# maybeLx/MVSFormerPlusPlus

Hardware: AMD Instinct MI355X
Metric: ref-views/sec at 1152x1536 N=5 D=192 4-stage; achieved HBM GB/s vs peak (higher is better)
Workload: dtype fp16 operands/storage, fp32 accumulate (every stage; 1-2 fp16 MFMA terms)

## Files before the change

### mvsformerplusplus_amd/csrc/conv_bf16x3_kernels.hip

```cpp
#include <map>
#include <mutex>
#include <type_traits>
#include <utility>

#include "conv_cfg.h"
#include "split_format.h"

namespace mvs {

template <class Base>
struct F16Cfg : Base { static constexpr int ACT_F16 = 1; };
template <class Base>
struct F16x1Cfg : Base { static constexpr int ACT_F16 = 2; };
template <class Cfg, class = void> struct CfgFmt { static constexpr bool F16 = false, ONE = false; };
template <class Cfg> struct CfgFmt<Cfg, decltype((void)Cfg::ACT_F16)> { static constexpr bool F16 = true, ONE = Cfg::ACT_F16 == 2; };
typedef _Float16 f16x8 __attribute__((ext_vector_type(8)));
typedef _Float16 f16x4 __attribute__((ext_vector_type(4)));

__device__ __forceinline__ f16x4 f16_pack4(const float4& v, float& amax) {
    const float m = 65504.0f;
    sat::track(amax, v.x, v.y, v.z, v.w);
    return f16x4{(_Float16)__builtin_amdgcn_fmed3f(v.x, -m, m), (_Float16)__builtin_amdgcn_fmed3f(v.y, -m, m),
                 (_Float16)__builtin_amdgcn_fmed3f(v.z, -m, m), (_Float16)__builtin_amdgcn_fmed3f(v.w, -m, m)};
}

__device__ __forceinline__ float4 f16_quad_to_f32(const float4& raw) {
    const float lo = raw.x, hi = raw.y;
    const f16x4 h = __builtin_bit_cast(f16x4, make_float2(lo, hi));
    return make_float4((float)h[0], (float)h[1], (float)h[2], (float)h[3]);
}

template <int MREP, int NREP, bool F16 = false, bool ONE = false>
__device__ __forceinline__ void bf_mfma_step(const bf16x8* ah, const bf16x8* al, const bf16x8* bh, const bf16x8* bl, f32x4 (*acc)[NREP]) {
    if constexpr (F16) {
        if constexpr (!ONE) {
#pragma unroll
            for (int mb = 0; mb < MREP; ++mb)
#pragma unroll
                for (int nb = 0; nb < NREP; ++nb)
                    acc[mb][nb] = __builtin_amdgcn_mfma_f32_16x16x32_f16(__builtin_bit_cast(f16x8, al[mb]), __builtin_bit_cast(f16x8, bh[nb]), acc[mb][nb], 0, 0, 0);
        }
#pragma unroll
        for (int mb = 0; mb < MREP; ++mb)
#pragma unroll
            for (int nb = 0; nb < NREP; ++nb)
                acc[mb][nb] = __builtin_amdgcn_mfma_f32_16x16x32_f16(__builtin_bit_cast(f16x8, ah[mb]), __builtin_bit_cast(f16x8, bh[nb]), acc[mb][nb], 0, 0, 0);
        return;
    }
#pragma unroll
    for (int mb = 0; mb < MREP; ++mb)
#pragma unroll
        for (int nb = 0; nb < NREP; ++nb) acc[mb][nb] = __builtin_amdgcn_mfma_f32_16x16x32_bf16(al[mb], bh[nb], acc[mb][nb], 0, 0, 0);
#pragma unroll
    for (int mb = 0; mb < MREP; ++mb)
#pragma unroll
        for (int nb = 0; nb < NREP; ++nb) acc[mb][nb] = __builtin_amdgcn_mfma_f32_16x16x32_bf16(ah[mb], bl[nb], acc[mb][nb], 0, 0, 0);
#pragma unroll
    for (int mb = 0; mb < MREP; ++mb)
#pragma unroll
        for (int nb = 0; nb < NREP; ++nb) acc[mb][nb] = __builtin_amdgcn_mfma_f32_16x16x32_bf16(ah[mb], bh[nb], acc[mb][nb], 0, 0, 0);
}

template <class Base, int MSPLIT_>
struct SplitCfg : Base {
    static constexpr int MSPLIT = MSPLIT_;
    static constexpr int MREP_ALL = Base::MREP;
    static constexpr int MREP = Base::MREP / MSPLIT_;
    static constexpr int NREP = Base::NREP * MSPLIT_;
    static_assert(Base::MREP % MSPLIT_ == 0 && 4 % MSPLIT_ == 0, "bad output-block split");
};
template <class Cfg, class = void> struct CfgSplit { static constexpr int MSPLIT = 1, MREP_ALL = Cfg::MREP; };
template <class Cfg> struct CfgSplit<Cfg, decltype((void)Cfg::MSPLIT)> { static constexpr int MSPLIT = Cfg::MSPLIT, MREP_ALL = Cfg::MREP_ALL; };

constexpr int bf_f16_plane_shift(int sw) { return sw == 1 ? 0 : 16; }

template <class Cfg>
struct BfConv {
    static constexpr int OPT = Cfg::CH / 8;
    static constexpr int NSTEP = (Cfg::NTAP * OPT + 3) / 4;
    static constexpr bool PLANES = OPT == 2;
    static constexpr bool F16 = CfgFmt<Cfg>::F16;
    static constexpr int RUNB = F16 ? 16 : 32;
    static constexpr int SB = F16 ? 16 : (PLANES ? 32 : Cfg::S * 4);
    static constexpr int PLANE = F16 ? (Cfg::NVOX * 16 + 255) / 256 * 256 + bf_f16_plane_shift(Cfg::SW)
                                     : (PLANES ? (Cfg::NVOX * 32 + 255) / 256 * 256 + 16 : 32);
    static constexpr size_t LDS_BYTES = F16 ? (size_t)OPT * PLANE : (PLANES ? (size_t)2 * PLANE : Cfg::LDS_BYTES);
    static constexpr bool ONE = CfgFmt<Cfg>::ONE;
    static constexpr bool PERSIST = (Cfg::CIN == 8 || ONE) && Cfg::NPASS == 1 && NSTEP * Cfg::MREP * (ONE ? 4 : 8) <= 64;
    static constexpr bool PERSIST_WLDS = PERSIST && ONE && Cfg::CIN == 16;
    static constexpr int WLDS_OFF = ((int)LDS_BYTES + 255) / 256 * 256;
    static constexpr size_t PERSIST_LDS_BYTES = PERSIST_WLDS ? (size_t)WLDS_OFF + (size_t)NSTEP * Cfg::MREP * 1024 : LDS_BYTES;
    static constexpr bool UNROLL_STAGE = !(Cfg::CIN == 32 && Cfg::COUT == 32);
    static_assert(Cfg::CH % 8 == 0 && OPT <= 2, "split-bf16 path stages one or two octets per pass");
};

constexpr unsigned BF_OOB = 0x80000000u;

__device__ __forceinline__ __amdgpu_buffer_rsrc_t bf_make_rsrc(const void* p, unsigned bytes) {
    return __builtin_amdgcn_make_buffer_rsrc(const_cast<void*>(p), 0, (int)bytes, 0x00020000);
}
__device__ __forceinline__ __amdgpu_buffer_rsrc_t bf_make_rsrc_z(const char* xb, int z0, int D, int H, int W, unsigned vstride, int& zrel) {
// ... 40 lines not shown
    const int tx = tile % tiles_x;
    const int t1 = tile / tiles_x;
    return {tx, t1 % tiles_y, t1 / tiles_y};
}

template <int MREP, int NREP>
__device__ __forceinline__ void bf_zero_acc(f32x4 (*acc)[NREP]) {
#pragma unroll
    for (int mb = 0; mb < MREP; ++mb)
#pragma unroll
        for (int nb = 0; nb < NREP; ++nb) acc[mb][nb] = (f32x4){0.0f, 0.0f, 0.0f, 0.0f};
}

template <bool F16, bool SPLIT>
__device__ __forceinline__ void bf_store_quad(float* o, int co, int g, const float4& v, bool ok, float& sat_amax) {
    static_assert(!(F16 && SPLIT), "fp16 tensors have no split form: only the split store looks at `ok`");
    if constexpr (F16) *reinterpret_cast<f16x4*>(reinterpret_cast<_Float16*>(o) + co) = f16_pack4(v, sat_amax);
    else if constexpr (SPLIT) split_store_quad(o + (co & ~7), g, v, ok);
    else *reinterpret_cast<float4*>(o + co) = v;
}
template <bool F16, bool SPLIT>
__device__ __forceinline__ void bf_skip_join(float4& v, const float4& raw) {
    const float4 sk = F16 ? f16_quad_to_f32(raw) : SPLIT ? split_join_quad(raw) : raw;
    v.x += sk.x; v.y += sk.y; v.z += sk.z; v.w += sk.w;
}
__device__ __forceinline__ void bf_prob_head(const float4& v, const float4& pw4, float pb, int g, bool ok, float* logits, size_t idx) {
    float part = v.x * pw4.x;
    part += v.y * pw4.y;
    part += v.z * pw4.z;
    part += v.w * pw4.w;
    part += __shfl_xor(part, 16);
    if ((g & 1) == 0 && ok) logits[idx] = part + pb;
}

template <class Cfg>
__device__ __forceinline__ constexpr int bf_tap_offset(int o) {
    constexpr int OPT = BfConv<Cfg>::OPT;
    int tap = o / OPT;
    const int oc = o - tap * OPT;
    tap = tap < Cfg::NTAP ? tap : Cfg::NTAP - 1;
    const int kd = tap / 9, r9 = tap - kd * 9, kh = r9 / 3, kw = r9 - kh * 3;
    return ((kd * Cfg::IH + kh) * Cfg::IW + kw) * BfConv<Cfg>::SB + oc * BfConv<Cfg>::PLANE;
}

template <class Cfg, int T>
__device__ __forceinline__ void bf_conv_load_w(const bf16x8* wq, bf16x8* ah, bf16x8* al) {
#pragma unroll
    for (int mb = 0; mb < Cfg::MREP; ++mb) {
        ah[mb] = wq[(size_t)((T * CfgSplit<Cfg>::MREP_ALL + mb) * 2) * 64];
        al[mb] = wq[(size_t)((T * CfgSplit<Cfg>::MREP_ALL + mb) * 2 + 1) * 64];
    }
}

template <class Cfg, int T>
__device__ __forceinline__ void bf_conv_load_x(int g, const char* ldsb, int voxbase0, bf16x8* bh, bf16x8* bl) {
    static_assert(Cfg::TH % Cfg::NREP == 0, "a wave's rows must stay inside one output plane");
    constexpr int ROWB = Cfg::SH * Cfg::IW * BfConv<Cfg>::SB;
    constexpr int c0 = bf_tap_offset<Cfg>(4 * T), c1 = bf_tap_offset<Cfg>(4 * T + 1), c2 = bf_tap_offset<Cfg>(4 * T + 2),
                  c3 = bf_tap_offset<Cfg>(4 * T + 3);
    int sel;
    if constexpr (BfConv<Cfg>::PLANES) {
        static_assert(c1 == c0 + BfConv<Cfg>::PLANE && c3 == c2 + BfConv<Cfg>::PLANE, "octet planes of one tap");
        sel = ((g & 2) ? c2 : c0) + (g & 1) * BfConv<Cfg>::PLANE;
    } else {
        sel = c0;
        sel = g == 1 ? c1 : sel;
        sel = g == 2 ? c2 : sel;
        sel = g == 3 ? c3 : sel;
    }
    const char* p = ldsb + voxbase0 + sel;
#pragma unroll
    for (int nb = 0; nb < Cfg::NREP; ++nb) {
        bh[nb] = *reinterpret_cast<const bf16x8*>(p + nb * ROWB);
        if constexpr (!BfConv<Cfg>::F16) bl[nb] = *reinterpret_cast<const bf16x8*>(p + nb * ROWB + 16);
    }
}

template <class Cfg, int T>
__device__ __forceinline__ void bf_conv_load_step(int g, const bf16x8* wq, const char* ldsb, int voxbase0, bf16x8* ah, bf16x8* al,
                                                  bf16x8* bh, bf16x8* bl) {
    bf_conv_load_w<Cfg, T>(wq, ah, al);
    bf_conv_load_x<Cfg, T>(g, ldsb, voxbase0, bh, bl);
}

constexpr int BF_WPF = 1;
template <class Cfg, int T>
struct BfConvSteps {
    static constexpr int WPF = BF_WPF, NW = WPF + 1;
    static __device__ __forceinline__ void run(int g, const bf16x8* wq, const char* ldsb, int voxbase0, f32x4 (*acc)[Cfg::NREP],
                                               bf16x8 (*ah)[Cfg::MREP], bf16x8 (*al)[Cfg::MREP], bf16x8* bh0, bf16x8* bl0, bf16x8* bh1, bf16x8* bl1) {
        constexpr int NSTEP = BfConv<Cfg>::NSTEP;
        if constexpr (T < NSTEP) {
            if constexpr (T + WPF < NSTEP) bf_conv_load_w<Cfg, T + WPF>(wq, ah[(T + WPF) % NW], al[(T + WPF) % NW]);
            if constexpr (T + 1 < NSTEP) {
                if constexpr ((T & 1) == 0) bf_conv_load_x<Cfg, T + 1>(g, ldsb, voxbase0, bh1, bl1);
                else bf_conv_load_x<Cfg, T + 1>(g, ldsb, voxbase0, bh0, bl0);
            }
            __builtin_amdgcn_sched_barrier(0);
            if constexpr ((T & 1) == 0) bf_mfma_step<Cfg::MREP, Cfg::NREP, CfgFmt<Cfg>::F16, CfgFmt<Cfg>::ONE>(ah[T % NW], al[T % NW], bh0, bl0, acc);
            else bf_mfma_step<Cfg::MREP, Cfg::NREP, CfgFmt<Cfg>::F16, CfgFmt<Cfg>::ONE>(ah[T % NW], al[T % NW], bh1, bl1, acc);
            BfConvSteps<Cfg, T + 1>::run(g, wq, ldsb, voxbase0, acc, ah, al, bh0, bl0, bh1, bl1);
        }
    }
};

template <class Cfg, int T = 0>
__device__ __forceinline__ void bf_conv_preload_w(const bf16x8* wq, bf16x8 (*ah)[Cfg::MREP], bf16x8 (*al)[Cfg::MREP]) {
    if constexpr (T < BF_WPF && T < BfConv<Cfg>::NSTEP) {
        bf_conv_load_w<Cfg, T>(wq, ah[T], al[T]);
        bf_conv_preload_w<Cfg, T + 1>(wq, ah, al);
    }
}

template <class Cfg>
__device__ __forceinline__ void bf_conv_contract(const bf16x8* wq, const char* ldsb, const int* voxbase, int g, f32x4 (*acc)[Cfg::NREP],
                                                 bf16x8 (*ah)[Cfg::MREP], bf16x8 (*al)[Cfg::MREP]) {
    constexpr int NREP = Cfg::NREP;
    bf16x8 bh0[NREP], bl0[NREP], bh1[NREP], bl1[NREP];
    bf_conv_load_x<Cfg, 0>(g, ldsb, voxbase[0], bh0, bl0);
    BfConvSteps<Cfg, 0>::run(g, wq, ldsb, voxbase[0], acc, ah, al, bh0, bl0, bh1, bl1);
}

template <class Cfg>
struct BfWlds {
    static constexpr int MREP_ALL = CfgSplit<Cfg>::MREP_ALL;
    static constexpr int NSTEP = BfConv<Cfg>::NSTEP;
    static constexpr int WC = (MREP_ALL == 1 && NSTEP % 2 == 0) ? 2 : 1;
    static constexpr int CHUNK_BYTES = WC * MREP_ALL * 2048;
    static constexpr int NPIECE = CHUNK_BYTES / 4096 > 0 ? CHUNK_BYTES / 4096 : 1;
    static constexpr int NCHUNK = NSTEP / WC;
    static constexpr int RING_OFF = ((int)BfConv<Cfg>::LDS_BYTES + 255) / 256 * 256;
    static constexpr size_t LDS_BYTES = (size_t)RING_OFF + 2 * CHUNK_BYTES;
    static constexpr bool ENABLED = !BfConv<Cfg>::PERSIST && NSTEP % WC == 0 && CHUNK_BYTES % 4096 == 0 && MREP_ALL == 1 && WC == 2;
};

struct BfWPiece { float4 a, b; };
template <class Cfg>
__device__ __forceinline__ void bf_wlds_fetch(const void* wp, int gc, int nchunk_total, int tid, BfWPiece& piece) {
    using W = BfWlds<Cfg>;
    static_assert(W::NPIECE <= 2, "at most two pieces per thread and chunk");
    if (gc >= nchunk_total) return;
    const float4* src = reinterpret_cast<const float4*>(reinterpret_cast<const char*>(wp) + (size_t)gc * W::CHUNK_BYTES);
    piece.a = src[tid];
    if constexpr (W::NPIECE > 1) piece.b = src[tid + 256];
}
template <class Cfg>
__device__ __forceinline__ void bf_wlds_store(char* ring, int gc, int tid, const BfWPiece& piece) {
    using W = BfWlds<Cfg>;
    float4* dst = reinterpret_cast<float4*>(ring + (gc & 1) * W::CHUNK_BYTES);
    dst[tid] = piece.a;
    if constexpr (W::NPIECE > 1) dst[tid + 256] = piece.b;
}

template <class Cfg, int T>
__device__ __forceinline__ void bf_wlds_load_a(const char* ring, int gc, int mb0, int lane, bf16x8* ah, bf16x8* al) {
    using W = BfWlds<Cfg>;
    const char* base = ring + (gc & 1) * W::CHUNK_BYTES + ((T % W::WC) * W::MREP_ALL + mb0) * 2048 + lane * 16;
#pragma unroll
    for (int mb = 0; mb < Cfg::MREP; ++mb) {
        ah[mb] = *reinterpret_cast<const bf16x8*>(base + mb * 2048);
        al[mb] = *reinterpret_cast<const bf16x8*>(base + mb * 2048 + 1024);
    }
}

template <class Cfg, int T>
struct BfWldsSteps {
    static __device__ __forceinline__ void run(int g, int lane, int tid, const void* wp, char* ring, int gc0, int nchunk_total, int mb0,
                                               const char* ldsb, int voxbase0, f32x4 (*acc)[Cfg::NREP], BfWPiece& piece, bf16x8* bh0, bf16x8* bl0,
                                               bf16x8* bh1, bf16x8* bl1) {
        using W = BfWlds<Cfg>;
        constexpr int NSTEP = W::NSTEP;
        if constexpr (T < NSTEP) {
            const int gc = gc0 + T / W::WC;
            if constexpr (T % W::WC == 0) bf_wlds_fetch<Cfg>(wp, gc + 1, nchunk_total, tid, piece);
            bf16x8 ah[Cfg::MREP], al[Cfg::MREP];
            bf_wlds_load_a<Cfg, T>(ring, gc, mb0, lane, ah, al);
            if constexpr (T + 1 < NSTEP) {
                if constexpr ((T & 1) == 0) bf_conv_load_x<Cfg, T + 1>(g, ldsb, voxbase0, bh1, bl1);
                else bf_conv_load_x<Cfg, T + 1>(g, ldsb, voxbase0, bh0, bl0);
            }
            __builtin_amdgcn_sched_barrier(0);
            if constexpr ((T & 1) == 0) bf_mfma_step<Cfg::MREP, Cfg::NREP, CfgFmt<Cfg>::F16, CfgFmt<Cfg>::ONE>(ah, al, bh0, bl0, acc);
            else bf_mfma_step<Cfg::MREP, Cfg::NREP, CfgFmt<Cfg>::F16, CfgFmt<Cfg>::ONE>(ah, al, bh1, bl1, acc);
            if constexpr (T % W::WC == W::WC - 1) {
                if (gc + 1 < nchunk_total) bf_wlds_store<Cfg>(ring, gc + 1, tid, piece);
                __syncthreads();
            }
            BfWldsSteps<Cfg, T + 1>::run(g, lane, tid, wp, ring, gc0, nchunk_total, mb0, ldsb, voxbase0, acc, piece, bh0, bl0, bh1, bl1);
        }
    }
};

template <class Cfg, bool SPLIT>
__global__ __launch_bounds__(256) void conv3d_mfma_bf16x3_kernel(const float* __restrict__ x, const void* wp, const float* __restrict__ bias,
                                                                 float* __restrict__ y, int D, int H, int W, int OD, int OH, int OW,
                                                                 int relu, int tiles_x, int tiles_y, int ntiles) {
    float sat_amax = 0.0f;
    constexpr int CIN = Cfg::CIN, COUT = Cfg::COUT, SD = Cfg::SD, SH = Cfg::SH, SW = Cfg::SW, TD = Cfg::TD, TH = Cfg::TH, CH = Cfg::CH;
    constexpr int IH = Cfg::IH, IW = Cfg::IW, MREP = Cfg::MREP, NREP = Cfg::NREP;
    constexpr int OPT = BfConv<Cfg>::OPT, NSTEP = BfConv<Cfg>::NSTEP, SB = BfConv<Cfg>::SB;
    HIP_DYNAMIC_SHARED(float4, lds4)
    char* ldsb = reinterpret_cast<char*>(lds4);
    const int tid = (int)threadIdx.x, lane = tid & 63, wave = tid >> 6;
    const int li = lane & 15, g = lane >> 4;
    const int tile = (int)xcd_remap(blockIdx.x, (unsigned)ntiles);
    const int b = (int)blockIdx.y;
    const BfTileOrigin t = bf_tile_origin(tile, tiles_x, tiles_y);
    const int oz0 = t.tz * TD, oy0 = t.ty * TH, ox0 = t.tx * 16;
    const int iz0 = oz0 * SD - Cfg::PD, iy0 = oy0 * SH - 1, ix0 = ox0 * SW - 1;

    f32x4 acc[MREP][NREP];
    bf_zero_acc<MREP, NREP>(acc);

    constexpr int MSPLIT = CfgSplit<Cfg>::MSPLIT, MREP_ALL = CfgSplit<Cfg>::MREP_ALL;
    const int mb0 = (wave % MSPLIT) * MREP, rowgrp = wave / MSPLIT;
    int voxbase[NREP];
#pragma unroll
    for (int nb = 0; nb < NREP; ++nb) {
        const int nbg = rowgrp * NREP + nb;
        const int oz = nbg / TH, oy = nbg % TH;
        voxbase[nb] = (((oz * SD) * IH + oy * SH) * IW + li * SW) * SB;
    }

    constexpr bool F16 = BfConv<Cfg>::F16;
    constexpr int EB = F16 ? 2 : 4, RUNB = BfConv<Cfg>::RUNB;
    const char* xb = reinterpret_cast<const char*>(x) + (size_t)b * D * H * W * CIN * EB;
    constexpr int NITEM = Cfg::NVOX * OPT, NIT = (NITEM + 255) / 256;
    float4 su[NIT], sv[NIT];
    int zrel;
    const __amdgpu_buffer_rsrc_t xrs = bf_make_rsrc_z(xb, iz0, D, H, W, (unsigned)(CIN * EB), zrel);
    auto issue = [&](int pass) {
        BfTileWalk<IW, IH, OPT, RUNB> wk(tid, zrel, iy0, ix0, H, W, CIN * EB, (unsigned)(pass * CH * EB));
#pragma unroll
        for (int it = 0; it < NIT; ++it) {
            if (it > 0) wk.advance();
            const bool ok = (it * 256 + 255 < NITEM || tid + it * 256 < NITEM) && wk.inside(iz0, iy0, ix0, D, H, W);
            const unsigned voff = ok ? wk.off : BF_OOB;
            su[it] = bf_buf_load16(xrs, voff, 0);
            if constexpr (!F16) sv[it] = bf_buf_load16(xrs, voff, 16);
        }
    };
// ... 23 lines not shown
        bf16x8 ah[BF_WPF + 1][MREP], al[BF_WPF + 1][MREP];
        if constexpr (!WLDS) bf_conv_preload_w<Cfg>(wq, ah, al);
        if (pass > 0 && !WLDS) __syncthreads();
        if constexpr (UNROLLED) {
            commit();
        } else {
            BfTileWalk<IW, IH, OPT, RUNB> wk(tid, zrel, iy0, ix0, H, W, CIN * EB, (unsigned)(pass * CH * EB));
            int ldso = (tid / OPT) * SB + (tid % OPT) * BfConv<Cfg>::PLANE;
#pragma unroll 1
            for (int e = tid; e < NITEM; e += 256) {
                const bool ok = wk.inside(iz0, iy0, ix0, D, H, W);
                const unsigned voff = ok ? wk.off : BF_OOB;
                const float4 u = bf_buf_load16(xrs, voff, 0);
                if constexpr (F16) {
                    *reinterpret_cast<float4*>(ldsb + ldso) = u;
                } else {
                    const float4 v = bf_buf_load16(xrs, voff, 16);
                    stage_to_lds<SPLIT>(ldsb + ldso, u, v);
                }
                wk.advance();
                ldso += (256 / OPT) * SB;
            }
        }
        __syncthreads();
        if (UNROLLED && pass + 1 < Cfg::NPASS) issue(pass + 1);
        if constexpr (WLDS) {
            bf16x8 bh0[NREP], bl0[NREP], bh1[NREP], bl1[NREP];
            bf_conv_load_x<Cfg, 0>(g, ldsb, voxbase[0], bh0, bl0);
            BfWldsSteps<Cfg, 0>::run(g, lane, tid, wp, ring, pass * BfWlds<Cfg>::NCHUNK, nchunk_total, mb0, ldsb, voxbase[0], acc, piece, bh0, bl0, bh1, bl1);
        } else {
            bf_conv_contract<Cfg>(wq, ldsb, voxbase, g, acc, ah, al);
        }
    }

    float* yb = reinterpret_cast<float*>(reinterpret_cast<char*>(y) + (size_t)b * OD * OH * OW * COUT * EB);
#pragma unroll
    for (int nb = 0; nb < NREP; ++nb) {
        const int nbg = rowgrp * NREP + nb;
        const int oz = oz0 + nbg / TH, oy = oy0 + nbg % TH, ox = ox0 + li;
        const bool inside = oz < OD && oy < OH && ox < OW;
        if (!SPLIT && !inside) continue;
        float* o = reinterpret_cast<float*>(reinterpret_cast<char*>(yb) + (((size_t)oz * OH + oy) * OW + ox) * COUT * EB);
#pragma unroll
        for (int mb = 0; mb < MREP; ++mb) {
            const int co = 16 * (mb0 + mb) + 4 * g;
            if (!SPLIT && co >= COUT) continue;
            const float4 bb = *reinterpret_cast<const float4*>(bias + (co < COUT ? co : 0));
            float4 v = make_float4(acc[mb][nb][0] + bb.x, acc[mb][nb][1] + bb.y, acc[mb][nb][2] + bb.z, acc[mb][nb][3] + bb.w);
            if (relu) { v.x = fmaxf(v.x, 0.0f); v.y = fmaxf(v.y, 0.0f); v.z = fmaxf(v.z, 0.0f); v.w = fmaxf(v.w, 0.0f); }
            bf_store_quad<F16, SPLIT>(o, co, g, v, inside && co < COUT, sat_amax);
        }
    }
    if constexpr (F16) sat::commit(sat_amax);
}


template <class Cfg, int T>
struct BfConvStepsWreg {
    static __device__ __forceinline__ void run(int g, const bf16x8 (*wh)[Cfg::MREP], const bf16x8 (*wl)[Cfg::MREP], const char* ldsb, int voxbase0,
                                               f32x4 (*acc)[Cfg::NREP], bf16x8* bh0, bf16x8* bl0, bf16x8* bh1, bf16x8* bl1, const char* wlane = nullptr) {
        constexpr int NSTEP = BfConv<Cfg>::NSTEP;
        if constexpr (T < NSTEP) {
            bf16x8 aw[Cfg::MREP];
            if constexpr (BfConv<Cfg>::PERSIST_WLDS) {
#pragma unroll
                for (int mb = 0; mb < Cfg::MREP; ++mb) aw[mb] = *reinterpret_cast<const bf16x8*>(wlane + (T * Cfg::MREP + mb) * 1024);
            }
            if constexpr (T + 1 < NSTEP) {
                if constexpr ((T & 1) == 0) bf_conv_load_x<Cfg, T + 1>(g, ldsb, voxbase0, bh1, bl1);
                else bf_conv_load_x<Cfg, T + 1>(g, ldsb, voxbase0, bh0, bl0);
            }
            __builtin_amdgcn_sched_barrier(0);
            const bf16x8* a_hi = BfConv<Cfg>::PERSIST_WLDS ? aw : wh[T];
            const bf16x8* a_lo = BfConv<Cfg>::PERSIST_WLDS ? aw : wl[T];
            if constexpr ((T & 1) == 0) bf_mfma_step<Cfg::MREP, Cfg::NREP, CfgFmt<Cfg>::F16, CfgFmt<Cfg>::ONE>(a_hi, a_lo, bh0, bl0, acc);
            else bf_mfma_step<Cfg::MREP, Cfg::NREP, CfgFmt<Cfg>::F16, CfgFmt<Cfg>::ONE>(a_hi, a_lo, bh1, bl1, acc);
            BfConvStepsWreg<Cfg, T + 1>::run(g, wh, wl, ldsb, voxbase0, acc, bh0, bl0, bh1, bl1, wlane);
        }
    }
};

template <class Cfg, bool SPLIT>
__global__ __launch_bounds__(256) void conv3d_mfma_bf16x3_persist_kernel(const float* __restrict__ x, const void* wp, const float* __restrict__ bias,
                                                                         float* __restrict__ y, float* __restrict__ logits, int D, int H, int W,
                                                                         int OD, int OH, int OW, int relu, int tiles_x, int tiles_y, int ntiles) {
    float sat_amax = 0.0f;
    constexpr int CIN = Cfg::CIN, COUT = Cfg::COUT, SD = Cfg::SD, SH = Cfg::SH, SW = Cfg::SW, TD = Cfg::TD, TH = Cfg::TH;
    constexpr int IH = Cfg::IH, IW = Cfg::IW, MREP = Cfg::MREP, NREP = Cfg::NREP;
    constexpr int OPT = BfConv<Cfg>::OPT, NSTEP = BfConv<Cfg>::NSTEP, SB = BfConv<Cfg>::SB;
    static_assert(Cfg::NPASS == 1, "the persistent form keeps one channel chunk's weights in registers");
    HIP_DYNAMIC_SHARED(float4, lds4)
    char* ldsb = reinterpret_cast<char*>(lds4);
    const int tid = (int)threadIdx.x, lane = tid & 63, wave = tid >> 6;
    const int li = lane & 15, g = lane >> 4;
    const int b = (int)blockIdx.y;
    const int nblk = (int)gridDim.x, per = (ntiles + nblk - 1) / nblk;
    const int t_begin = (int)xcd_remap(blockIdx.x, (unsigned)nblk) * per;
    const int t_end = t_begin + per < ntiles ? t_begin + per : ntiles;
    if (t_begin >= t_end) return;

    const bf16x8* wq = reinterpret_cast<const bf16x8*>(wp) + lane;
    bf16x8 wh[NSTEP][MREP], wl[NSTEP][MREP];
    constexpr bool WL = BfConv<Cfg>::PERSIST_WLDS;
    const char* wlane = ldsb + BfConv<Cfg>::WLDS_OFF + lane * 16;
    if constexpr (WL) {
        bf16x8* dst = reinterpret_cast<bf16x8*>(ldsb + BfConv<Cfg>::WLDS_OFF);
// ... 587 lines not shown
                const bool inside = mz < D && my < H && mx < W;
                const int oz = mz * SD + pd, oy = 2 * my + ph, ox = 2 * mx + (g >> 1);
                float4 v = outv[it][nb];
                if (sb) bf_skip_join<F16, SPLIT>(v, skp[it][nb]);
                if (head) {
                    bf_prob_head(v, pw4, pb, g, inside, logits, (size_t)b * OD * OH * OW + ((size_t)oz * OH + oy) * OW + ox);
                } else if (SPLIT || inside) {
                    float* o = reinterpret_cast<float*>(reinterpret_cast<char*>(yb) + (((size_t)oz * OH + oy) * OW + ox) * COUT * EB);
                    bf_store_quad<F16, SPLIT>(o, co, g, v, inside, sat_amax);
                }
            }
        }
        if (sb && tile + 1 < t_end) issue_skip(tile + 1);
        __syncthreads();
    }
    if constexpr (F16) sat::commit(sat_amax);
}

static int resident_blocks(const void* func, size_t lds, int threads = 256) {
    static std::mutex mu;
    static std::map<std::pair<const void*, int>, int> cache;
    int dev = 0;
    if (hipGetDevice(&dev) != hipSuccess) return -1;
    std::lock_guard<std::mutex> lock(mu);
    auto it = cache.find(std::make_pair(func, dev));
    if (it != cache.end()) return it->second;
    int per_cu = 0;
    hipDeviceProp_t prop;
    if (lds > 48 * 1024) hipFuncSetAttribute(func, hipFuncAttributeMaxDynamicSharedMemorySize, (int)lds);
    if (hipGetDeviceProperties(&prop, dev) != hipSuccess || hipOccupancyMaxActiveBlocksPerMultiprocessor(&per_cu, func, threads, lds) != hipSuccess || per_cu < 1)
        return -1;
    return cache[std::make_pair(func, dev)] = per_cu * prop.multiProcessorCount;
}

static int bf_persist_grid(const void* func, size_t lds, int ntiles) {
    const int resident = resident_blocks(func, lds);
    return resident < 1 ? 0 : (ntiles < resident ? ntiles : resident);
}

template <class... KArgs, class... Args>
static int bf_launch(void (*kernel)(KArgs...), const char* name, dim3 grid, size_t lds, hipStream_t st, Args... args) {
    if (lds > 48 * 1024) hipFuncSetAttribute(reinterpret_cast<const void*>(kernel), hipFuncAttributeMaxDynamicSharedMemorySize, (int)lds);
    hipLaunchKernelGGL(kernel, grid, dim3(256), lds, st, args...);
    return check_launch(name);
}

constexpr int BF_MSPLIT_MIN_MREP = 4;
template <class Cfg>
struct BfSplitOf {
    static constexpr bool SPLIT = Cfg::MREP >= BF_MSPLIT_MIN_MREP && Cfg::NREP <= 2 && Cfg::TH % (Cfg::NREP * 2) == 0;
    typedef typename std::conditional<SPLIT, SplitCfg<Cfg, 2>, Cfg>::type type;
};

template <class Cfg, bool SPLIT>
static int launch_conv_bf(const float* x, const void* wp, const float* bias, float* y, int B, int D, int H, int W, int relu, hipStream_t st,
                          float* logits) {
    const int OD = (D + 2 * Cfg::PD - Cfg::KD) / Cfg::SD + 1, OH = (H - 1) / Cfg::SH + 1, OW = (W - 1) / Cfg::SW + 1;
    const int tx = (int)ceil_div(OW, 16), ty = (int)ceil_div(OH, Cfg::TH), tz = (int)ceil_div(OD, Cfg::TD);
    const int ntiles = tx * ty * tz;
    constexpr size_t LDS = BfConv<Cfg>::PERSIST ? BfConv<Cfg>::PERSIST_LDS_BYTES : BfConv<Cfg>::LDS_BYTES;
    if constexpr (BfConv<Cfg>::PERSIST) {
        const int nblk = bf_persist_grid(reinterpret_cast<const void*>(&conv3d_mfma_bf16x3_persist_kernel<Cfg, SPLIT>), LDS, ntiles);
        if (nblk < 1) { set_error("conv3d(bf16x3): occupancy query failed"); return MVS_ERR_LAUNCH; }
        return bf_launch(&conv3d_mfma_bf16x3_persist_kernel<Cfg, SPLIT>, "conv3d_mfma_bf16x3_persist_kernel", dim3(nblk, B), LDS, st, x, wp, bias, y, logits, D, H,
                         W, OD, OH, OW, relu, tx, ty, ntiles);
    } else {
        if (logits != nullptr) { set_error("conv3d(bf16x3): the planar single-channel output needs a persistent (Cin = 8) kernel"); return MVS_ERR_UNSUPPORTED; }
        constexpr size_t TLDS = BfWlds<Cfg>::ENABLED ? BfWlds<Cfg>::LDS_BYTES : LDS;
        return bf_launch(&conv3d_mfma_bf16x3_kernel<Cfg, SPLIT>, "conv3d_mfma_bf16x3_kernel", dim3(ntiles, B), TLDS, st, x, wp, bias, y, D, H, W, OD, OH, OW, relu, tx,
                         ty, ntiles);
    }
}

template <class Cfg>
struct BfDeconvSplitOf {
    static constexpr bool SPLIT = Cfg::MREP == 2 && Cfg::THM % (Cfg::NREP * 2) == 0;
    typedef typename std::conditional<SPLIT, SplitCfg<Cfg, 2>, Cfg>::type type;
};

template <class Cfg, bool SPLIT>
static int launch_deconv_bf(const float* x, const void* wp, const float* bias, const float* skip, float* y, const float* prob_w,
                            const float* prob_b, float* logits, int B, int D, int H, int W, hipStream_t st, int relu) {
    const int tx = (int)ceil_div(W, 16), ty = (int)ceil_div(H, Cfg::THM), tz = (int)ceil_div(D, Cfg::TDM);
    const int ntiles = tx * ty * tz;
    if constexpr (Cfg::CIN == 16 && Cfg::COUT == 8) {
        constexpr size_t LDS = BfDeconvP<Cfg>::LDS_BYTES;
        const int nblk = bf_persist_grid(reinterpret_cast<const void*>(&deconv3d_mfma_bf16x3_persist_kernel<Cfg, SPLIT>), LDS, ntiles);
        if (nblk < 1) { set_error("deconv3d(bf16x3): occupancy query failed"); return MVS_ERR_LAUNCH; }
        return bf_launch(&deconv3d_mfma_bf16x3_persist_kernel<Cfg, SPLIT>, "deconv3d_mfma_bf16x3_persist_kernel", dim3(nblk, B), LDS, st, x, wp, bias, skip, y,
                         prob_w, prob_b, logits, D, H, W, tx, ty, ntiles, relu);
    } else {
        constexpr size_t DLDS = BfDeconv<Cfg>::LDS_BYTES;
        if constexpr (BfDeconvF<Cfg>::ENABLED) {
            const char* sw = getenv("MVS_DECONV_CLASS_FUSED");
            const bool fused = (sw == nullptr || sw[0] == '\0') ? BfDeconvF<Cfg>::DEFAULT : sw[0] != '0';
            if (fused)
                return bf_launch(&deconv3d_mfma_bf16x3_kernel<Cfg, SPLIT, true>, "deconv3d_mfma_bf16x3_kernel", dim3(ntiles, B), DLDS, st, x, wp, bias, skip, y, D, H, W,
                                 tx, ty, ntiles, relu);
        }
        return bf_launch(&deconv3d_mfma_bf16x3_kernel<Cfg, SPLIT, false>, "deconv3d_mfma_bf16x3_kernel", dim3(ntiles, B), DLDS, st, x, wp, bias, skip, y, D, H, W, tx, ty,
                         ntiles, relu);
    }
}

static bool bf_input_fits(const char* who, int Cin, int D, int H, int W, int split) {
    const long long bytes = 12LL * H * W * Cin * (split >= 2 ? 2 : 4);
    if (bytes < (1LL << 31)) return true;
    set_error("%s: twelve z-planes of the input are %lld bytes; the MFMA convolutions address a tile's planes with 32-bit offsets (< 2 GB)", who, bytes);
    return false;
}

int conv3d_dispatch_bf16x3(const float* x, const void* wp, const float* bias, float* y, int B, int Cin, int Cout, int D, int H, int W,
                           int kd, int sd, int sh, int sw, int relu, hipStream_t st, float* logits, int split) {
    if (!bf_input_fits("conv3d(mfma)", Cin, D, H, W, split)) return MVS_ERR_UNSUPPORTED;
#define MVS_X(CI, CO, KD, SD, SH, SW, TD, TH, CH)                                                     \
    if (Cin == CI && Cout == CO && kd == KD && sd == SD && sh == SH && sw == SW) {                    \
        typedef typename BfSplitOf<ConvCfg<CI, CO, KD, SD, SH, SW, TD, TH, CH>>::type K;              \
        if (split == 3) return launch_conv_bf<F16x1Cfg<K>, false>(x, wp, bias, y, B, D, H, W, relu, st, logits); \
        if (split == 2) return launch_conv_bf<F16Cfg<K>, false>(x, wp, bias, y, B, D, H, W, relu, st, logits);   \
        return split ? launch_conv_bf<K, true>(x, wp, bias, y, B, D, H, W, relu, st, logits)          \
                     : launch_conv_bf<K, false>(x, wp, bias, y, B, D, H, W, relu, st, logits);        \
// ... 29 lines not shown
```

Baseline: 694.0.

## Skip zero-padded depth taps in fp16 3D conv edge tiles

Adds a specialized fp16 conv3d kernel for depth-shallow layers that classifies tiles touching the low or high depth boundary. For those tiles it skips loading the padded input plane, drops MFMAs for output rows whose taps are all padding, and points partially padded octets at a zeroed LDS strip. The goal is to cut wasted MFMA and load work from depth padding when D is small. It adds template instantiations per edge class, a different row-to-wave mapping, and a debug counter plus an environment switch.

```diff
diff --git a/mvsformerplusplus_amd/csrc/conv_bf16x3_kernels.hip b/mvsformerplusplus_amd/csrc/conv_bf16x3_kernels.hip
--- a/mvsformerplusplus_amd/csrc/conv_bf16x3_kernels.hip
+++ b/mvsformerplusplus_amd/csrc/conv_bf16x3_kernels.hip
@@ -1,3 +1,4 @@
+#include <atomic>
 #include <map>
 #include <mutex>
 #include <type_traits>
@@ -30,8 +31,24 @@
     return make_float4((float)h[0], (float)h[1], (float)h[2], (float)h[3]);
 }
 
-template <int MREP, int NREP, bool F16 = false, bool ONE = false>
+template <int MREP, int NREP, unsigned MASK, int NB = 0>
+__device__ __forceinline__ void bf_mfma_rows(const bf16x8* a, const bf16x8* bh, f32x4 (*acc)[NREP]) {
+    if constexpr (NB < MREP * NREP) {
+        constexpr int mb = NB / NREP, nb = NB % NREP;
+        if constexpr (((MASK >> nb) & 1u) != 0)
+            acc[mb][nb] = __builtin_amdgcn_mfma_f32_16x16x32_f16(__builtin_bit_cast(f16x8, a[mb]), __builtin_bit_cast(f16x8, bh[nb]), acc[mb][nb], 0, 0, 0);
+        bf_mfma_rows<MREP, NREP, MASK, NB + 1>(a, bh, acc);
+    }
+}
+
+template <int MREP, int NREP, bool F16 = false, bool ONE = false, unsigned MASK = ~0u>
 __device__ __forceinline__ void bf_mfma_step(const bf16x8* ah, const bf16x8* al, const bf16x8* bh, const bf16x8* bl, f32x4 (*acc)[NREP]) {
+    if constexpr (MASK != ~0u) {
+        static_assert(F16, "row masks: fp16 activation formats only");
+        if constexpr (!ONE) bf_mfma_rows<MREP, NREP, MASK>(al, bh, acc);
+        bf_mfma_rows<MREP, NREP, MASK>(ah, bh, acc);
+        return;
+    }
     if constexpr (F16) {
         if constexpr (!ONE) {
 #pragma unroll
@@ -47,6 +64,7 @@
                 acc[mb][nb] = __builtin_amdgcn_mfma_f32_16x16x32_f16(__builtin_bit_cast(f16x8, ah[mb]), __builtin_bit_cast(f16x8, bh[nb]), acc[mb][nb], 0, 0, 0);
         return;
     }
+    static_assert(F16 || MASK == ~0u, "row masks: fp16 activation formats only");
 #pragma unroll
     for (int mb = 0; mb < MREP; ++mb)
 #pragma unroll
@@ -193,9 +211,46 @@
     }
 }
 
-template <class Cfg, int T>
-__device__ __forceinline__ void bf_conv_load_x(int g, const char* ldsb, int voxbase0, bf16x8* bh, bf16x8* bl) {
-    static_assert(Cfg::TH % Cfg::NREP == 0, "a wave's rows must stay inside one output plane");
+template <class Cfg>
+struct BfZEdgeOf {
+    static constexpr bool AVAILABLE = BfConv<Cfg>::F16 && !BfConv<Cfg>::PERSIST && Cfg::KD == 3 && Cfg::SD == 1 && Cfg::NREP % Cfg::TD == 0;
+    static constexpr int DEFAULT_MAX_D = !AVAILABLE ? 0
+        : (Cfg::CIN == 16 && Cfg::COUT == 16 && !CfgFmt<Cfg>::ONE) || (Cfg::CIN == 32 && Cfg::COUT == 32 && CfgFmt<Cfg>::ONE) ? 8
+        : (Cfg::CIN == 16 && Cfg::COUT == 32 && !CfgFmt<Cfg>::ONE) ? 4 : 0;
+};
+template <class Cfg, int ZE>
+struct BfZEdge {
+    static constexpr bool LOW = (ZE & 1) != 0, HIGH = (ZE & 2) != 0;
+    static constexpr int TD = Cfg::TD, NREP = Cfg::NREP, OPT = BfConv<Cfg>::OPT;
+    static_assert(ZE == 0 || BfZEdgeOf<Cfg>::AVAILABLE, "no z-edge body for this tile configuration");
+    static constexpr int YPW = ZE ? NREP / TD : 1;
+    static constexpr int PLB = Cfg::IH * Cfg::IW * BfConv<Cfg>::SB;
+    static constexpr int dz(int nb) { return ZE ? nb % TD : 0; }
+    static constexpr int dy(int nb) { return ZE ? nb / TD : nb; }
+    static constexpr int rowoff(int nb) { return dz(nb) * PLB + dy(nb) * Cfg::SH * Cfg::IW * BfConv<Cfg>::SB; }
+    static constexpr int Z0 = LOW ? 1 : 0, NZ = Cfg::ID - (LOW ? 1 : 0) - (HIGH ? 1 : 0);
+    static constexpr int STRIP = (LOW ? 0 : Cfg::ID - 1) * PLB;
+    static constexpr bool octet_ok(int nb, int o) {
+        int tap = o / OPT;
+        tap = tap < Cfg::NTAP ? tap : Cfg::NTAP - 1;
+        const int kd = tap / 9;
+        return !(LOW && dz(nb) == 0 && kd == 0) && !(HIGH && dz(nb) == TD - 1 && kd == 2);
+    }
+    static constexpr unsigned bad_groups(int nb, int T) {
+        unsigned m = 0;
+        for (int gg = 0; gg < 4; ++gg) m |= octet_ok(nb, 4 * T + gg) ? 0u : 1u << gg;
+        return m;
+    }
+    static constexpr unsigned rows(int T) {
+        unsigned m = 0;
+        for (int nb = 0; nb < NREP; ++nb) m |= bad_groups(nb, T) == 15u ? 0u : 1u << nb;
+        return ZE ? m : ~0u;
+    }
+};
+
+template <class Cfg, int T, int ZE = 0>
+__device__ __forceinline__ void bf_conv_load_x(int g, const char* ldsb, int voxbase0, bf16x8* bh, bf16x8* bl, const char* zs = nullptr) {
+    static_assert(ZE != 0 || Cfg::TH % Cfg::NREP == 0, "a wave's rows must stay inside one output plane");
     constexpr int ROWB = Cfg::SH * Cfg::IW * BfConv<Cfg>::SB;
     constexpr int c0 = bf_tap_offset<Cfg>(4 * T), c1 = bf_tap_offset<Cfg>(4 * T + 1), c2 = bf_tap_offset<Cfg>(4 * T + 2),
                   c3 = bf_tap_offset<Cfg>(4 * T + 3);
@@ -210,6 +265,18 @@
         sel = g == 3 ? c3 : sel;
     }
     const char* p = ldsb + voxbase0 + sel;
+    if constexpr (ZE != 0) {
+        using Z = BfZEdge<Cfg, ZE>;
+#pragma unroll
+        for (int nb = 0; nb < Cfg::NREP; ++nb) {
+            const unsigned bad = Z::bad_groups(nb, T);
+            if (bad == 15u) continue;
+            const char* q = p + Z::rowoff(nb);
+            if (bad != 0u) q = ((bad >> g) & 1u) ? zs : q;
+            bh[nb] = *reinterpret_cast<const bf16x8*>(q);
+        }
+        return;
+    }
 #pragma unroll
     for (int nb = 0; nb < Cfg::NREP; ++nb) {
         bh[nb] = *reinterpret_cast<const bf16x8*>(p + nb * ROWB);
@@ -225,22 +292,24 @@
 }
 
 constexpr int BF_WPF = 1;
-template <class Cfg, int T>
+template <class Cfg, int T, int ZE = 0>
 struct BfConvSteps {
     static constexpr int WPF = BF_WPF, NW = WPF + 1;
     static __device__ __forceinline__ void run(int g, const bf16x8* wq, const char* ldsb, int voxbase0, f32x4 (*acc)[Cfg::NREP],
-                                               bf16x8 (*ah)[Cfg::MREP], bf16x8 (*al)[Cfg::MREP], bf16x8* bh0, bf16x8* bl0, bf16x8* bh1, bf16x8* bl1) {
+                                               bf16x8 (*ah)[Cfg::MREP], bf16x8 (*al)[Cfg::MREP], bf16x8* bh0, bf16x8* bl0, bf16x8* bh1, bf16x8* bl1,
+                                               const char* zs = nullptr) {
         constexpr int NSTEP = BfConv<Cfg>::NSTEP;
         if constexpr (T < NSTEP) {
+            constexpr unsigned ROWS = BfZEdge<Cfg, ZE>::rows(T);
             if constexpr (T + WPF < NSTEP) bf_conv_load_w<Cfg, T + WPF>(wq, ah[(T + WPF) % NW], al[(T + WPF) % NW]);
             if constexpr (T + 1 < NSTEP) {
-                if constexpr ((T & 1) == 0) bf_conv_load_x<Cfg, T + 1>(g, ldsb, voxbase0, bh1, bl1);
-                else bf_conv_load_x<Cfg, T + 1>(g, ldsb, voxbase0, bh0, bl0);
+                if constexpr ((T & 1) == 0) bf_conv_load_x<Cfg, T + 1, ZE>(g, ldsb, voxbase0, bh1, bl1, zs);
+                else bf_conv_load_x<Cfg, T + 1, ZE>(g, ldsb, voxbase0, bh0, bl0, zs);
             }
             __builtin_amdgcn_sched_barrier(0);
-            if constexpr ((T & 1) == 0) bf_mfma_step<Cfg::MREP, Cfg::NREP, CfgFmt<Cfg>::F16, CfgFmt<Cfg>::ONE>(ah[T % NW], al[T % NW], bh0, bl0, acc);
-            else bf_mfma_step<Cfg::MREP, Cfg::NREP, CfgFmt<Cfg>::F16, CfgFmt<Cfg>::ONE>(ah[T % NW], al[T % NW], bh1, bl1, acc);
-            BfConvSteps<Cfg, T + 1>::run(g, wq, ldsb, voxbase0, acc, ah, al, bh0, bl0, bh1, bl1);
+            if constexpr ((T & 1) == 0) bf_mfma_step<Cfg::MREP, Cfg::NREP, CfgFmt<Cfg>::F16, CfgFmt<Cfg>::ONE, ROWS>(ah[T % NW], al[T % NW], bh0, bl0, acc);
+            else bf_mfma_step<Cfg::MREP, Cfg::NREP, CfgFmt<Cfg>::F16, CfgFmt<Cfg>::ONE, ROWS>(ah[T % NW], al[T % NW], bh1, bl1, acc);
+            BfConvSteps<Cfg, T + 1, ZE>::run(g, wq, ldsb, voxbase0, acc, ah, al, bh0, bl0, bh1, bl1, zs);
         }
     }
 };
@@ -253,13 +322,13 @@
     }
 }
 
-template <class Cfg>
+template <class Cfg, int ZE = 0>
 __device__ __forceinline__ void bf_conv_contract(const bf16x8* wq, const char* ldsb, const int* voxbase, int g, f32x4 (*acc)[Cfg::NREP],
-                                                 bf16x8 (*ah)[Cfg::MREP], bf16x8 (*al)[Cfg::MREP]) {
+                                                 bf16x8 (*ah)[Cfg::MREP], bf16x8 (*al)[Cfg::MREP], const char* zs = nullptr) {
     constexpr int NREP = Cfg::NREP;
     bf16x8 bh0[NREP], bl0[NREP], bh1[NREP], bl1[NREP];
-    bf_conv_load_x<Cfg, 0>(g, ldsb, voxbase[0], bh0, bl0);
-    BfConvSteps<Cfg, 0>::run(g, wq, ldsb, voxbase[0], acc, ah, al, bh0, bl0, bh1, bl1);
+    bf_conv_load_x<Cfg, 0, ZE>(g, ldsb, voxbase[0], bh0, bl0, zs);
+    BfConvSteps<Cfg, 0, ZE>::run(g, wq, ldsb, voxbase[0], acc, ah, al, bh0, bl0, bh1, bl1, zs);
 }
 
 template <class Cfg>
@@ -304,11 +373,12 @@
     }
 }
 
-template <class Cfg, int T>
+template <class Cfg, int T, int ZE = 0>
 struct BfWldsSteps {
     static __device__ __forceinline__ void run(int g, int lane, int tid, const void* wp, char* ring, int gc0, int nchunk_total, int mb0,
                                                const char* ldsb, int voxbase0, f32x4 (*acc)[Cfg::NREP], BfWPiece& piece, bf16x8* bh0, bf16x8* bl0,
-                                               bf16x8* bh1, bf16x8* bl1) {
+                                               bf16x8* bh1, bf16x8* bl1, const char* zs = nullptr) {
+        constexpr unsigned ROWS = BfZEdge<Cfg, ZE>::rows(T < BfWlds<Cfg>::NSTEP ? T : 0);
         using W = BfWlds<Cfg>;
         constexpr int NSTEP = W::NSTEP;
         if constexpr (T < NSTEP) {
@@ -317,17 +387,17 @@
             bf16x8 ah[Cfg::MREP], al[Cfg::MREP];
             bf_wlds_load_a<Cfg, T>(ring, gc, mb0, lane, ah, al);
             if constexpr (T + 1 < NSTEP) {
-                if constexpr ((T & 1) == 0) bf_conv_load_x<Cfg, T + 1>(g, ldsb, voxbase0, bh1, bl1);
-                else bf_conv_load_x<Cfg, T + 1>(g, ldsb, voxbase0, bh0, bl0);
+                if constexpr ((T & 1) == 0) bf_conv_load_x<Cfg, T + 1, ZE>(g, ldsb, voxbase0, bh1, bl1, zs);
+                else bf_conv_load_x<Cfg, T + 1, ZE>(g, ldsb, voxbase0, bh0, bl0, zs);
             }
             __builtin_amdgcn_sched_barrier(0);
-            if constexpr ((T & 1) == 0) bf_mfma_step<Cfg::MREP, Cfg::NREP, CfgFmt<Cfg>::F16, CfgFmt<Cfg>::ONE>(ah, al, bh0, bl0, acc);
-            else bf_mfma_step<Cfg::MREP, Cfg::NREP, CfgFmt<Cfg>::F16, CfgFmt<Cfg>::ONE>(ah, al, bh1, bl1, acc);
+            if constexpr ((T & 1) == 0) bf_mfma_step<Cfg::MREP, Cfg::NREP, CfgFmt<Cfg>::F16, CfgFmt<Cfg>::ONE, ROWS>(ah, al, bh0, bl0, acc);
+            else bf_mfma_step<Cfg::MREP, Cfg::NREP, CfgFmt<Cfg>::F16, CfgFmt<Cfg>::ONE, ROWS>(ah, al, bh1, bl1, acc);
             if constexpr (T % W::WC == W::WC - 1) {
                 if (gc + 1 < nchunk_total) bf_wlds_store<Cfg>(ring, gc + 1, tid, piece);
                 __syncthreads();
             }
-            BfWldsSteps<Cfg, T + 1>::run(g, lane, tid, wp, ring, gc0, nchunk_total, mb0, ldsb, voxbase0, acc, piece, bh0, bl0, bh1, bl1);
+            BfWldsSteps<Cfg, T + 1, ZE>::run(g, lane, tid, wp, ring, gc0, nchunk_total, mb0, ldsb, voxbase0, acc, piece, bh0, bl0, bh1, bl1, zs);
         }
     }
 };
@@ -457,6 +527,135 @@
         }
     }
     if constexpr (F16) sat::commit(sat_amax);
+}
+
+__host__ __device__ __forceinline__ int bf_zedge_class(int oz0, int TD, int OD) {
+    return oz0 + TD > OD ? 0 : (oz0 == 0 ? 1 : 0) | (oz0 + TD == OD ? 2 : 0);
+}
+
+template <class Cfg>
+__global__ __launch_bounds__(256) void conv3d_mfma_f16_zedge_kernel(const float* __restrict__ x, const void* wp, const float* __restrict__ bias,
+                                                                    float* __restrict__ y, int D, int H, int W, int OD, int OH, int OW,
+                                                                    int relu, int tiles_x, int tiles_y, int ntiles) {
+    static_assert(BfZEdgeOf<Cfg>::AVAILABLE, "z-edge bodies: fp16 3x3x3 layers without depth stride");
+    HIP_DYNAMIC_SHARED(float4, lds4)
+    char* ldsb = reinterpret_cast<char*>(lds4);
+    const int tile = (int)xcd_remap(blockIdx.x, (unsigned)ntiles);
+    const BfTileOrigin t = bf_tile_origin(tile, tiles_x, tiles_y);
+    auto tile_body = [&](auto zec) __attribute__((always_inline)) {
+        constexpr int ZE = decltype(zec)::value;
+        using Z = BfZEdge<Cfg, ZE>;
+        float sat_amax = 0.0f;
+        constexpr int CIN = Cfg::CIN, COUT = Cfg::COUT, SH = Cfg::SH, SW = Cfg::SW, TD = Cfg::TD, TH = Cfg::TH, CH = Cfg::CH;
+        constexpr int IH = Cfg::IH, IW = Cfg::IW, MREP = Cfg::MREP, NREP = Cfg::NREP;
+        constexpr int OPT = BfConv<Cfg>::OPT, NSTEP = BfConv<Cfg>::NSTEP, SB = BfConv<Cfg>::SB, PLANE = BfConv<Cfg>::PLANE;
+        const int tid = (int)threadIdx.x, lane = tid & 63, wave = tid >> 6;
+        const int li = lane & 15, g = lane >> 4;
+        const int b = (int)blockIdx.y;
+        const int oz0 = t.tz * TD, oy0 = t.ty * TH, ox0 = t.tx * 16;
+        const int iz0 = oz0 - 1 + Z::Z0, iy0 = oy0 * SH - 1, ix0 = ox0 * SW - 1;
+
+        f32x4 acc[MREP][NREP];
+        bf_zero_acc<MREP, NREP>(acc);
+
+        constexpr int MSPLIT = CfgSplit<Cfg>::MSPLIT, MREP_ALL = CfgSplit<Cfg>::MREP_ALL;
+        const int mb0 = (wave % MSPLIT) * MREP, rowgrp = wave / MSPLIT;
+        auto row_z = [&](int nb) { return ZE ? Z::dz(nb) : (rowgrp * NREP + nb) / TH; };
+        auto row_y = [&](int nb) { return ZE ? rowgrp * Z::YPW + Z::dy(nb) : (rowgrp * NREP + nb) % TH; };
+        int voxbase[1] = {((row_z(0) * IH + row_y(0) * SH) * IW + li * SW) * SB};
+        const char* zs = nullptr;
+        if constexpr (ZE != 0) {
+            if (tid < 16 * OPT) *reinterpret_cast<float4*>(ldsb + Z::STRIP + (tid & 15) * SB + (tid >> 4) * PLANE) = make_float4(0.0f, 0.0f, 0.0f, 0.0f);
+            zs = ldsb + Z::STRIP + li * SB + (OPT == 2 ? (g & 1) * PLANE : 0);
+        }
+
+        const char* xb = reinterpret_cast<const char*>(x) + (size_t)b * D * H * W * CIN * 2;
+        constexpr int LDS0 = Z::Z0 * Z::PLB;
+        constexpr int NITEM = Z::NZ * IH * IW * OPT, NIT = (NITEM + 255) / 256;
+        float4 su[NIT];
+        int zrel;
+        const __amdgpu_buffer_rsrc_t xrs = bf_make_rsrc_z(xb, iz0, D, H, W, (unsigned)(CIN * 2), zrel);
+        auto issue = [&](int pass) {
+            BfTileWalk<IW, IH, OPT, 16> wk(tid, zrel, iy0, ix0, H, W, CIN * 2, (unsigned)(pass * CH * 2));
+#pragma unroll
+            for (int it = 0; it < NIT; ++it) {
+                if (it > 0) wk.advance();
+                const bool ok = (it * 256 + 255 < NITEM || tid + it * 256 < NITEM) && wk.inside(iz0, iy0, ix0, D, H, W);
+                su[it] = bf_buf_load16(xrs, ok ? wk.off : BF_OOB, 0);
+            }
+        };
+        auto commit = [&]() {
+#pragma unroll
+            for (int it = 0; it < NIT; ++it) {
+                const int e = tid + it * 256;
+                if (e >= NITEM) break;
+                const int vox = e / OPT, oc = e - vox * OPT;
+                *reinterpret_cast<float4*>(ldsb + LDS0 + vox * SB + oc * PLANE) = su[it];
+            }
+        };
+        constexpr bool UNROLLED = BfConv<Cfg>::UNROLL_STAGE;
+        constexpr bool WLDS = BfWlds<Cfg>::ENABLED;
+        char* ring = ldsb + BfWlds<Cfg>::RING_OFF;
+        constexpr int nchunk_total = Cfg::NPASS * BfWlds<Cfg>::NCHUNK;
+        BfWPiece piece;
+        piece.a = piece.b = make_float4(0.0f, 0.0f, 0.0f, 0.0f);
+        if constexpr (WLDS) bf_wlds_fetch<Cfg>(wp, 0, nchunk_total, tid, piece);
+        if constexpr (UNROLLED) issue(0);
+        if constexpr (WLDS) bf_wlds_store<Cfg>(ring, 0, tid, piece);
+        for (int pass = 0; pass < Cfg::NPASS; ++pass) {
+            const bf16x8* wq = reinterpret_cast<const bf16x8*>(wp) + ((size_t)pass * NSTEP * MREP_ALL + mb0) * 2 * 64 + lane;
+            bf16x8 ah[BF_WPF + 1][MREP], al[BF_WPF + 1][MREP];
+            if constexpr (!WLDS) bf_conv_preload_w<Cfg>(wq, ah, al);
+            if (pass > 0 && !WLDS) __syncthreads();
+            if constexpr (UNROLLED) {
+                commit();
+            } else {
+                BfTileWalk<IW, IH, OPT, 16> wk(tid, zrel, iy0, ix0, H, W, CIN * 2, (unsigned)(pass * CH * 2));
+                int ldso = LDS0 + (tid / OPT) * SB + (tid % OPT) * PLANE;
+#pragma unroll 1
+                for (int e = tid; e < NITEM; e += 256) {
+                    const bool ok = wk.inside(iz0, iy0, ix0, D, H, W);
+                    *reinterpret_cast<float4*>(ldsb + ldso) = bf_buf_load16(xrs, ok ? wk.off : BF_OOB, 0);
+                    wk.advance();
+                    ldso += (256 / OPT) * SB;
+                }
+            }
+            __syncthreads();
+            if (UNROLLED && pass + 1 < Cfg::NPASS) issue(pass + 1);
+            if constexpr (WLDS) {
+                bf16x8 bh0[NREP], bh1[NREP];
+                bf_conv_load_x<Cfg, 0, ZE>(g, ldsb, voxbase[0], bh0, nullptr, zs);
+                BfWldsSteps<Cfg, 0, ZE>::run(g, lane, tid, wp, ring, pass * BfWlds<Cfg>::NCHUNK, nchunk_total, mb0, ldsb, voxbase[0], acc, piece, bh0, nullptr, bh1,
+                                             nullptr, zs);
+            } else {
+                bf_conv_contract<Cfg, ZE>(wq, ldsb, voxbase, g, acc, ah, al, zs);
+            }
+        }
+
+        char* yb = reinterpret_cast<char*>(y) + (size_t)b * OD * OH * OW * COUT * 2;
+#pragma unroll
+        for (int nb = 0; nb < NREP; ++nb) {
+            const int oz = oz0 + row_z(nb), oy = oy0 + row_y(nb), ox = ox0 + li;
+            if (!(oz < OD && oy < OH && ox < OW)) continue;
+            float* o = reinterpret_cast<float*>(yb + (((size_t)oz * OH + oy) * OW + ox) * COUT * 2);
+#pragma unroll
+            for (int mb = 0; mb < MREP; ++mb) {
+                const int co = 16 * (mb0 + mb) + 4 * g;
+                if (co >= COUT) continue;
+                const float4 bb = *reinterpret_cast<const float4*>(bias + co);
+                float4 v = make_float4(acc[mb][nb][0] + bb.x, acc[mb][nb][1] + bb.y, acc[mb][nb][2] + bb.z, acc[mb][nb][3] + bb.w);
+                if (relu) { v.x = fmaxf(v.x, 0.0f); v.y = fmaxf(v.y, 0.0f); v.z = fmaxf(v.z, 0.0f); v.w = fmaxf(v.w, 0.0f); }
+                bf_store_quad<true, false>(o, co, g, v, true, sat_amax);
+            }
+        }
+        sat::commit(sat_amax);
+    };
+    switch (bf_zedge_class(t.tz * Cfg::TD, Cfg::TD, OD)) {
+        case 1: tile_body(std::integral_constant<int, 1>{}); break;
+        case 2: tile_body(std::integral_constant<int, 2>{}); break;
+        case 3: tile_body(std::integral_constant<int, 3>{}); break;
+        default: tile_body(std::integral_constant<int, 0>{}); break;
+    }
 }
 
 
@@ -1150,6 +1349,9 @@
     typedef typename std::conditional<SPLIT, SplitCfg<Cfg, 2>, Cfg>::type type;
 };
 
+static std::atomic<unsigned long long> g_zedge_tiles{0};
+extern "C" __attribute__((visibility("default"))) unsigned long long mvs_debug_conv_zedge_tiles() { return g_zedge_tiles.load(); }
+
 template <class Cfg, bool SPLIT>
 static int launch_conv_bf(const float* x, const void* wp, const float* bias, float* y, int B, int D, int H, int W, int relu, hipStream_t st,
                           float* logits) {
@@ -1165,6 +1367,17 @@
     } else {
         if (logits != nullptr) { set_error("conv3d(bf16x3): the planar single-channel output needs a persistent (Cin = 8) kernel"); return MVS_ERR_UNSUPPORTED; }
         constexpr size_t TLDS = BfWlds<Cfg>::ENABLED ? BfWlds<Cfg>::LDS_BYTES : LDS;
+        if constexpr (BfZEdgeOf<Cfg>::AVAILABLE) {
+            const char* sw = getenv("MVS_CONV_ZEDGE");
+            const bool zedge = (sw == nullptr || sw[0] == '\0') ? D <= BfZEdgeOf<Cfg>::DEFAULT_MAX_D : sw[0] != '0';
+            if (zedge) {
+                long long edge_planes = 0;
+                for (int z = 0; z < tz; ++z) edge_planes += bf_zedge_class(z * Cfg::TD, Cfg::TD, OD) != 0;
+                g_zedge_tiles += (unsigned long long)(edge_planes * tx * ty * B);
+                return bf_launch(&conv3d_mfma_f16_zedge_kernel<Cfg>, "conv3d_mfma_f16_zedge_kernel", dim3(ntiles, B), TLDS, st, x, wp, bias, y, D, H, W, OD, OH, OW,
+                                 relu, tx, ty, ntiles);
+            }
+        }
         return bf_launch(&conv3d_mfma_bf16x3_kernel<Cfg, SPLIT>, "conv3d_mfma_bf16x3_kernel", dim3(ntiles, B), TLDS, st, x, wp, bias, y, D, H, W, OD, OH, OW, relu, tx,
                          ty, ntiles);
     }
```

After: 695.2, median of 3. About the same (+0.2%).
